# DK-Jang/MOCHA_SIGASIA2023

Hardware: AMD Instinct MI355X
Metric: characterized frames/sec (whole node) at T=60, 22 joints; 1/2/4/8 GPU (higher is better)
Workload: dtype f32; 1 GPU; demo pair (BASELINE configs[1]): 585 src x 585 cha windows, T=60, V=22, C=15, bank build + encode/match/decode/to_mot per step (characterize_pair); windows_per_gpu=585, joints=22, bank_entries=585, parallelism=dp1 (independent windows, no in-step collective)

## Files before the change

### mocha_sigasia2023_amd/csrc/gemm_x3.hip

```cpp
#include "kernels.h"
#include "device_utils.h"
#include <type_traits>
#include <algorithm>

namespace mocha {

typedef float f32x16 __attribute__((ext_vector_type(16)));
typedef float f32x4 __attribute__((ext_vector_type(4)));
typedef short s16x8 __attribute__((ext_vector_type(8)));
typedef unsigned int u32x2 __attribute__((ext_vector_type(2)));
typedef unsigned int u32x4 __attribute__((ext_vector_type(4)));

#ifndef X3_MAXSUM
#define X3_MAXSUM 2
#endif
static constexpr int XN = 128, XK = 16;
static constexpr int XA_HALF = 128 * 8 + 32;
static constexpr int XA_PLANE = 2 * XA_HALF;
static constexpr int XB_PLANE = 128 * 16;
static constexpr int XB_OFF = 3 * XA_PLANE;
static constexpr int X_STAGE = XB_OFF + 3 * XA_PLANE;
static constexpr int XW_BLOCK = 3 * XB_PLANE;
template <int TN> struct XT {
    static constexpr int TILE_N = 64 * TN;
    static constexpr int B_HALF = TILE_N * 8 + 32;
    static constexpr int B_PLANE = 2 * B_HALF;
    static constexpr int STAGE = XB_OFF + 3 * B_PLANE;
};
static_assert(XT<2>::STAGE == X_STAGE && XT<2>::B_HALF == XA_HALF, "TN = 2 is the 128-wide layout");

__device__ __forceinline__ float x3_lrelu(float x) { return x > 0.f ? x : 0.2f * x; }
__device__ __forceinline__ float x3_gelu(float x) { return mocha_gelu(x); }

__global__ __launch_bounds__(256) void mocha_pack_x3(const float* __restrict__ W, const float* __restrict__ wsub, int N, int K, unsigned short* __restrict__ out) {
    const int ksteps = K / XK;
    const int nt = blockIdx.x / ksteps, ks = blockIdx.x - nt * ksteps;
    const int r = threadIdx.x >> 1, h = threadIdx.x & 1;
    const int n = nt * XN + r;
    const int k = ks * XK + 8 * h;
    f32x4 lo = {0.f, 0.f, 0.f, 0.f}, hi = lo;
    if (n < N) {
        lo = *reinterpret_cast<const f32x4*>(W + (size_t)n * K + k);
        hi = *reinterpret_cast<const f32x4*>(W + (size_t)n * K + k + 4);
        if (wsub) {
            lo -= *reinterpret_cast<const f32x4*>(wsub + k);
            hi -= *reinterpret_cast<const f32x4*>(wsub + k + 4);
        }
    }
    u32x2 a[3], b[3];
    plane_split4(lo, a); plane_split4(hi, b);
    unsigned short* blk = out + (size_t)blockIdx.x * XW_BLOCK;
#pragma unroll
    for (int q = 0; q < 3; ++q) {
        const u32x4 v = {a[q][0], a[q][1], b[q][0], b[q][1]};
        *reinterpret_cast<u32x4*>(blk + q * XB_PLANE + h * 1024 + r * 8) = v;
    }
}

size_t gemm_x3_packed_elems(int N, int K) { return (size_t)((N + XN - 1) / XN) * (K / XK) * XW_BLOCK; }

hipError_t launch_pack_x3(const float* W, int N, int K, unsigned short* out, hipStream_t s, const float* wsub) {
    if (K % XK != 0) return hipErrorInvalidValue;
    const long long blocks = (long long)((N + XN - 1) / XN) * (K / XK);
    if (blocks > 0x7fffffffll) return hipErrorInvalidValue;
    hipLaunchKernelGGL(mocha_pack_x3, dim3((unsigned)blocks), dim3(256), 0, s, W, wsub, N, K, out);
    return hipGetLastError();
}

template <bool LRELU, bool GATHER, int TM, int TN>
__global__ __launch_bounds__(256) __attribute__((amdgpu_waves_per_eu(3, 3))) void mocha_gemm_x3(GemmParams p) {
    constexpr int TILE_M = TM * 64;
    constexpr int TILE_N = XT<TN>::TILE_N, B_HALF = XT<TN>::B_HALF, B_PLANE = XT<TN>::B_PLANE, STAGE = XT<TN>::STAGE;
    extern __shared__ __attribute__((aligned(16))) unsigned short x3_sm[];
    const int tid = threadIdx.x;
    const int lane = tid & 63, wave = tid >> 6;
    const int l31 = lane & 31, hh = lane >> 5;
    const int wm = wave >> 1, wn = wave & 1;

    const int n_tiles = (p.N + TILE_N - 1) / TILE_N;
    const int m_tiles = (p.M + TILE_M - 1) / TILE_M;
    const int bid = blockIdx.x;
    int mt, nt;
    if (m_tiles >= 8) {
        const int grp = bid / (8 * n_tiles);
        const int rem = bid - grp * 8 * n_tiles;
        mt = grp * 8 + (rem & 7);
        nt = rem >> 3;
    } else {
        mt = bid / n_tiles;
        nt = bid - mt * n_tiles;
    }
    if (mt >= m_tiles) return;
    const int m0 = mt * TILE_M, n0 = nt * TILE_N;
    const int steps_total = p.K / XK;
    const int per = (steps_total + p.ksplit - 1) / p.ksplit;
    const int s0 = blockIdx.z * per;
    const int nsteps = (s0 + per) <= steps_total ? per : steps_total - s0;
#ifdef X3_EXP_STAMPS
    long long stamp[4];
    stamp[3] = (long long)__builtin_amdgcn_s_memrealtime();
    stamp[0] = (long long)__builtin_amdgcn_s_memtime();
#define X3_STAMP(i) stamp[i] = (long long)__builtin_amdgcn_s_memtime()
#define X3_STAMP_OUT() do { if (tid == 0) { long long* d = (long long*)p.wsub + (size_t)bid * 6; d[0] = stamp[0]; d[1] = stamp[1]; d[2] = stamp[2]; d[3] = (long long)__builtin_amdgcn_s_memtime(); d[4] = stamp[3]; d[5] = (long long)__builtin_amdgcn_s_memrealtime(); } } while (0)
#else
#define X3_STAMP(i)
#define X3_STAMP_OUT()
#endif

    const int lrow = tid >> 2;
    const int lc = tid & 3;
    const __amdgpu_buffer_rsrc_t rsA = make_rsrc(GATHER ? p.A : p.A + (size_t)(m0 < p.M ? m0 : 0) * p.lda);
    int a_rb[TM], a_t[TM];
    unsigned a_off[TM];
#pragma unroll
    for (int i = 0; i < TM; ++i) {
        int m = m0 + lrow + 64 * i;
        m = m < p.M ? m : p.M - 1;
        if (GATHER) {
            const int v = m % p.V;
            const int bt = m / p.V;
            a_t[i] = bt % p.T_out;
            a_rb[i] = (bt / p.T_out) * p.T_src * p.V + v;
            a_off[i] = 0;
        } else {
            a_rb[i] = m; a_t[i] = 0;
            a_off[i] = ((unsigned)(m - m0) * (unsigned)p.lda + lc * 4) * 4u;
        }
    }
    f32x4 rset[2][TM];
    auto load_a = [&](int s, f32x4 (&ra)[TM]) __attribute__((always_inline)) {
        const int k0 = (s0 + s) * XK;
        if (!GATHER) {
#pragma unroll
            for (int i = 0; i < TM; ++i) ra[i] = bload(rsA, a_off[i], (unsigned)k0 * 4u);
        } else {
            const int tap = k0 / p.Cc;
            const int cin = k0 - tap * p.Cc;
#pragma unroll
            for (int i = 0; i < TM; ++i) {
                int tf = a_t[i] * p.stride + tap * p.tstep - p.pad;
                tf = tf < 0 ? -tf : tf;
                tf = tf >= p.T_full ? 2 * (p.T_full - 1) - tf : tf;
                const unsigned off = ((unsigned)(a_rb[i] + (tf >> p.tshift) * p.V) * (unsigned)p.lda + lc * 4) * 4u;
                ra[i] = bload(rsA, off, (unsigned)cin * 4u);
            }
        }
    };
    const int a_wr = (lc >> 1) * XA_HALF + lrow * 8 + (lc & 1) * 4;
    auto split_store = [&](const f32x4 (&ra)[TM], unsigned short* st) __attribute__((always_inline)) {
#pragma unroll
        for (int i = 0; i < TM; ++i) {
            f32x4 v = ra[i];
            if (LRELU) { v[0] = x3_lrelu(v[0]); v[1] = x3_lrelu(v[1]); v[2] = x3_lrelu(v[2]); v[3] = x3_lrelu(v[3]); }
            u32x2 pl[3];
            plane_split4(v, pl);
#pragma unroll
            for (int q = 0; q < 3; ++q) *reinterpret_cast<u32x2*>(st + q * XA_PLANE + a_wr + i * 64 * 8) = pl[q];
        }
    };
    const int wblock = TN == 1 ? nt >> 1 : nt;
    const __amdgpu_buffer_rsrc_t rsW = make_rsrc(p.Wsplit + ((size_t)wblock * steps_total + s0) * XW_BLOCK);
    auto dma_w = [&](int s, unsigned short* st) __attribute__((always_inline)) {
        if (TN == 2) {
#pragma unroll
            for (int j = 0; j < 3; ++j)
                __builtin_amdgcn_raw_ptr_buffer_load_lds(rsW, (__attribute__((address_space(3))) void*)(st + XB_OFF + ((j * 4 + wave) >> 2) * B_PLANE +
                                                         (((j * 4 + wave) >> 1) & 1) * B_HALF + ((j * 4 + wave) & 1) * 512), 16,
                                                         (unsigned)(j * 256 + tid) * 16u, (unsigned)s * (XW_BLOCK * 2u), 0, 0);
        } else {
#pragma unroll
            for (int j = 0; j < 2; ++j) {
                const int pc = j * 4 + wave;
                if (pc < 6)
                    __builtin_amdgcn_raw_ptr_buffer_load_lds(rsW, (__attribute__((address_space(3))) void*)(st + XB_OFF + (pc >> 1) * B_PLANE + (pc & 1) * B_HALF), 16,
                                                             (unsigned)(((pc >> 1) * 4 + (pc & 1) * 2 + (nt & 1)) * 64 + lane) * 16u, (unsigned)s * (XW_BLOCK * 2u), 0, 0);
            }
        }
    };

    f32x16 acc[TM][TN];
#pragma unroll
    for (int i = 0; i < TM; ++i)
#pragma unroll
        for (int j = 0; j < TN; ++j)
#pragma unroll
            for (int r = 0; r < 16; ++r) acc[i][j][r] = 0.f;

    const int fa = hh * XA_HALF + (wm * TM * 32 + l31) * 8;
    const int fb = XB_OFF + hh * B_HALF + (wn * 32 * TN + l31) * 8;

    load_a(0, rset[0]);
    __builtin_amdgcn_sched_barrier(0);
    dma_w(0, x3_sm);
    __builtin_amdgcn_sched_barrier(0);
    split_store(rset[0], x3_sm);
    load_a(1, rset[1]);
    __builtin_amdgcn_sched_barrier(0);
    asm volatile("s_waitcnt vmcnt(%0) lgkmcnt(0)\n\ts_barrier" ::"n"(TM) : "memory");

    auto step = [&](int s, auto parity, auto fetch_w, auto fetch_a) __attribute__((always_inline)) {
        constexpr bool FETCH_W = decltype(fetch_w)::value, FETCH_A = decltype(fetch_a)::value;
        constexpr int P = decltype(parity)::value;
        unsigned short* cur = x3_sm + P * STAGE;
        unsigned short* nxt = x3_sm + (P ^ 1) * STAGE;
        if (FETCH_W) dma_w(s + 1, nxt);
        __builtin_amdgcn_sched_barrier(0);
        if (FETCH_A) load_a(s + 2, rset[P]);
        __builtin_amdgcn_sched_barrier(0);
        s16x8 a[3][TM], b[3][TN];
        auto rd_a = [&](int q) __attribute__((always_inline)) {
#pragma unroll
            for (int i = 0; i < TM; ++i) a[q][i] = *reinterpret_cast<const s16x8*>(cur + q * XA_PLANE + fa + i * 32 * 8);
        };
        auto rd_b = [&](int q) __attribute__((always_inline)) {
#pragma unroll
            for (int i = 0; i < TN; ++i) b[q][i] = *reinterpret_cast<const s16x8*>(cur + q * B_PLANE + fb + i * 32 * 8);
        };
        rd_a(0); rd_b(2); rd_a(1); rd_b(1); rd_a(2); rd_b(0);
        float x[4 * TM];
        unsigned pk[2 * TM][3], hi[2 * TM][2];
        if (FETCH_W) {
#pragma unroll
            for (int e = 0; e < 4 * TM; ++e) { x[e] = rset[P ^ 1][e >> 2][e & 3]; if (LRELU) x[e] = fmaxf(x[e], 0.2f * x[e]); }
        }
        auto split_op = [&](int k) __attribute__((always_inline)) {
            const int pr = k / 11, o = k % 11, lvl = o / 5;
            float& x0 = x[2 * pr]; float& x1 = x[2 * pr + 1];
            if (o == 10) { pk[pr][2] = cvt_pk_bf16(x0, x1); return; }
            switch (o % 5) {
                case 0: pk[pr][lvl] = cvt_pk_bf16(x0, x1); break;
                case 1: hi[pr][0] = pk[pr][lvl] << 16; break;
                case 2: hi[pr][1] = pk[pr][lvl] & 0xffff0000u; break;
                case 3: x0 -= __uint_as_float(hi[pr][0]); break;
                default: x1 -= __uint_as_float(hi[pr][1]); break;
            }
        };
        auto write_row = [&](int i) __attribute__((always_inline)) {
#pragma unroll
            for (int q = 0; q < 3; ++q) {
                const u32x2 v = {pk[2 * i][q], pk[2 * i + 1][q]};
                *reinterpret_cast<u32x2*>(nxt + q * XA_PLANE + a_wr + i * 64 * 8) = v;
            }
        };
        __builtin_amdgcn_sched_barrier(0);
#pragma unroll
        for (int m = 0; m < 6 * TM * TN; ++m) {
            const int pr = m / (TM * TN), pa = PLANE_PA[pr], pb = PLANE_PB[pr], i = (m % (TM * TN)) / TN, j = m % TN;
            if (X3_MAXSUM == 2 || pr == 5)
                acc[i][j] = __builtin_amdgcn_mfma_f32_32x32x16_bf16(b[pb][j], a[pa][i], acc[i][j], 0, 0, 0);
            if (TN == 2) {
                if (FETCH_W && m < 11 * TM) { split_op(2 * m); split_op(2 * m + 1); }
                if (FETCH_W && m == 10) write_row(0);
                if (FETCH_W && TM == 2 && m == 21) write_row(1);
            } else if (TM == 1) {
                if (FETCH_W) {
#pragma unroll
                    for (int k = 4 * m; k < 4 * m + 4; ++k)
                        if (k < 22) split_op(k);
                }
                if (FETCH_W && m == 5) write_row(0);
            } else {
                if (FETCH_W && m < 11) { split_op(4 * m); split_op(4 * m + 1); split_op(4 * m + 2); split_op(4 * m + 3); }
                if (FETCH_W && m == 5) write_row(0);
                if (FETCH_W && m == 10) write_row(1);
            }
            __builtin_amdgcn_sched_barrier(0);
        }
        if (FETCH_A) asm volatile("s_waitcnt vmcnt(%0) lgkmcnt(0)\n\ts_barrier" ::"n"(TM) : "memory");
        else asm volatile("s_waitcnt vmcnt(0) lgkmcnt(0)\n\ts_barrier" ::: "memory");
    };
    X3_STAMP(1);
    using T = std::true_type; using F = std::false_type;
    using P0 = std::integral_constant<int, 0>; using P1 = std::integral_constant<int, 1>;
    for (int s = 0; s + 2 < nsteps; s += 2) {
        step(s, P0{}, T{}, T{});
        step(s + 1, P1{}, T{}, T{});
    }
    step(nsteps - 2, P0{}, T{}, F{});
    step(nsteps - 1, P1{}, F{}, F{});
    X3_STAMP(2);

    const bool vec_ok = ((p.ldc & 3) == 0) && (!p.residual || (p.ldr & 3) == 0) && ((p.N & 3) == 0);
    float* Cz = p.C + (size_t)blockIdx.z * p.slab_stride;
    const __amdgpu_buffer_rsrc_t rsC = make_rsrc(Cz + (size_t)m0 * p.ldc + n0);
    const __amdgpu_buffer_rsrc_t rsBias = make_rsrc(p.bias ? p.bias + n0 : p.A);
    const __amdgpu_buffer_rsrc_t rsRb = make_rsrc(p.rowbias ? p.rowbias + n0 : p.A);
    const __amdgpu_buffer_rsrc_t rsRes = make_rsrc(p.residual ? p.residual + (size_t)m0 * p.ldr + n0 : p.A);

    if (vec_ok && n0 + TILE_N <= p.N) {
        constexpr int LDP = TILE_N + 4;
        constexpr int C4 = TILE_N / 4;
        static_assert(64 * LDP * 4 <= 2 * STAGE * 2, "epilogue staging fits the operand stages");
        float* stage = reinterpret_cast<float*>(x3_sm);
        static_assert(256 % C4 == 0, "a thread keeps its column quad over the iterations");
        constexpr int NIT = 64 * C4 / 256, RSTEP = 256 / C4;
        const int c4 = tid % C4, r0 = tid / C4;
        const unsigned cb = (unsigned)c4 * 16u;
        const f32x4 zero4 = {0.f, 0.f, 0.f, 0.f};
        const f32x4 bias4 = p.bias ? bload(rsBias, cb, 0u) : zero4;
        const bool pre_res = p.residual != nullptr, pre_rb = !pre_res && p.rowbias != nullptr;
        f32x4 pre[2];
        auto fetch_pre = [&](int k) __attribute__((always_inline)) {
            const int rloc = 64 * (k / NIT) + r0 + RSTEP * (k % NIT);
            int row = m0 + rloc;
            row = row < p.M ? row : p.M - 1;
            if (pre_res) pre[k & 1] = bload(rsRes, (unsigned)(row - m0) * (unsigned)p.ldr * 4u + cb, 0u);
            else if (pre_rb) pre[k & 1] = bload(rsRb, (unsigned)(row % p.rb_mod) * (unsigned)p.N * 4u + cb, 0u);
        };
        if (pre_res || pre_rb) { fetch_pre(0); fetch_pre(1); }
        const bool plain_out = !p.bias && !p.rowbias && !p.residual;
#pragma unroll
        for (int h = 0; h < TM; ++h) {
#pragma unroll
            for (int i = 0; i < TM; ++i) {
                const int rblk = wm * TM + i;
                if ((rblk >> 1) != h) continue;
                float* srow = stage + ((rblk & 1) * 32 + l31) * LDP + wn * (32 * TN) + 4 * hh;
#pragma unroll
                for (int j = 0; j < TN; ++j)
#pragma unroll
                    for (int g = 0; g < 4; ++g) {
                        f32x4 v = {acc[i][j][4 * g], acc[i][j][4 * g + 1], acc[i][j][4 * g + 2], acc[i][j][4 * g + 3]};
                        *reinterpret_cast<f32x4*>(srow + j * 32 + 8 * g) = v;
                    }
            }
            __syncthreads();
            if (plain_out) {
#pragma unroll
                for (int it = 0; it < NIT; ++it) {
                    const int r = r0 + RSTEP * it;
                    const int rloc = 64 * h + r;
                    if (m0 + rloc < p.M) {
                        f32x4 v = *reinterpret_cast<const f32x4*>(stage + r * LDP + c4 * 4);
                        if (p.act == 1) { v = mocha_gelu4(v); }
                        else if (p.act == 2) { v[0] = x3_lrelu(v[0]); v[1] = x3_lrelu(v[1]); v[2] = x3_lrelu(v[2]); v[3] = x3_lrelu(v[3]); }
                        else if (p.act == 3) { v[0] = fmaxf(v[0], 0.f); v[1] = fmaxf(v[1], 0.f); v[2] = fmaxf(v[2], 0.f); v[3] = fmaxf(v[3], 0.f); }
                        bstore(rsC, v, (unsigned)rloc * (unsigned)p.ldc * 4u + cb, 0u);
                    }
                }
            } else
#pragma unroll
            for (int it = 0; it < NIT; ++it) {
                const int r = r0 + RSTEP * it;
                const int rloc = 64 * h + r;
                f32x4 v = *reinterpret_cast<const f32x4*>(stage + r * LDP + c4 * 4) + bias4;
                if (pre_rb) v += pre[(NIT * h + it) & 1];
                else if (p.rowbias) v += bload(rsRb, (unsigned)((m0 + rloc) % p.rb_mod) * (unsigned)p.N * 4u + cb, 0u);
                if (p.act == 1) { v = mocha_gelu4(v); }
                else if (p.act == 2) { v[0] = x3_lrelu(v[0]); v[1] = x3_lrelu(v[1]); v[2] = x3_lrelu(v[2]); v[3] = x3_lrelu(v[3]); }
                else if (p.act == 3) { v[0] = fmaxf(v[0], 0.f); v[1] = fmaxf(v[1], 0.f); v[2] = fmaxf(v[2], 0.f); v[3] = fmaxf(v[3], 0.f); }
                if (pre_res) v += pre[(NIT * h + it) & 1];
                if ((pre_res || pre_rb) && NIT * h + it + 2 < NIT * TM) fetch_pre(NIT * h + it + 2);
                if (m0 + rloc < p.M) bstore(rsC, v, (unsigned)rloc * (unsigned)p.ldc * 4u + cb, 0u);
            }
            if (h + 1 < TM) __syncthreads();
        }
        X3_STAMP_OUT();
        return;
    }

#pragma unroll
    for (int i = 0; i < TM; ++i) {
        const int row = m0 + (wm * TM + i) * 32 + l31;
        if (row >= p.M) continue;
        const float* rbrow = p.rowbias ? p.rowbias + (size_t)(row % p.rb_mod) * p.N : nullptr;
        const float* rsrow = p.residual ? p.residual + (size_t)row * p.ldr : nullptr;
        float* crow = Cz + (size_t)row * p.ldc;
#pragma unroll
        for (int j = 0; j < TN; ++j)
#pragma unroll
            for (int g = 0; g < 4; ++g)
#pragma unroll
                for (int e = 0; e < 4; ++e) {
                    const int c1 = n0 + wn * (32 * TN) + j * 32 + 8 * g + 4 * hh + e;
                    if (c1 >= p.N) continue;
                    float x = acc[i][j][4 * g + e];
                    if (p.bias) x += p.bias[c1];
                    if (rbrow) x += rbrow[c1];
                    if (p.act == 1) x = x3_gelu(x);
                    else if (p.act == 2) x = x3_lrelu(x);
                    else if (p.act == 3) x = fmaxf(x, 0.f);
                    if (rsrow) x += rsrow[c1];
                    crow[c1] = x;
                }
    }
}


template <bool LRELU, bool GATHER, int EPI>
__global__ __launch_bounds__(256) __attribute__((amdgpu_waves_per_eu(3, 3))) void mocha_gemm_x3p(GemmParams p) {
    constexpr int TM = 2, TN = 2;
    constexpr int TILE_M = 128, TILE_N = 128, B_HALF = XT<2>::B_HALF, B_PLANE = XT<2>::B_PLANE, STAGE = XT<2>::STAGE;
    extern __shared__ __attribute__((aligned(16))) unsigned short x3_sm[];
    const int tid = threadIdx.x;
    const int lane = tid & 63, wave = tid >> 6;
    const int l31 = lane & 31, hh = lane >> 5;
    const int wm = wave >> 1, wn = wave & 1;
    const int n_tiles = (p.N + TILE_N - 1) / TILE_N;
    const int m_tiles = (p.M + TILE_M - 1) / TILE_M;
    const int m_pad = m_tiles >= 8 ? (m_tiles + 7) / 8 * 8 : m_tiles;
    const int total = m_pad * n_tiles;
    const int nsteps = p.K / XK;
    const int lrow = tid >> 2, lc = tid & 3;

    struct Tile { int m0, n0; int valid; int a_rb[TM], a_t[TM]; unsigned a_off[TM]; };
    auto make_tile = [&](int t) __attribute__((always_inline)) -> Tile {
        Tile T;
        int mt, nt;
        if (m_tiles >= 8) {
            const int grp = t / (8 * n_tiles);
            const int rem = t - grp * 8 * n_tiles;
            mt = grp * 8 + (rem & 7);
            nt = rem >> 3;
        } else {
            mt = t / n_tiles;
            nt = t - mt * n_tiles;
        }
        T.valid = mt < m_tiles;
        T.m0 = (T.valid ? mt : 0) * TILE_M; T.n0 = nt * TILE_N;
#pragma unroll
        for (int i = 0; i < TM; ++i) {
            int m = T.m0 + lrow + 64 * i;
            m = m < p.M ? m : p.M - 1;
            if (GATHER) {
                const int v = m % p.V;
                const int bt = m / p.V;
                T.a_t[i] = bt % p.T_out;
                T.a_rb[i] = (bt / p.T_out) * p.T_src * p.V + v;
                T.a_off[i] = 0;
            } else {
                T.a_rb[i] = m; T.a_t[i] = 0;
                T.a_off[i] = ((unsigned)(m - T.m0) * (unsigned)p.lda + lc * 4) * 4u;
            }
        }
        return T;
    };
    f32x4 rset[2][TM];
    auto load_a = [&](const Tile& T, int s, f32x4 (&ra)[TM]) __attribute__((always_inline)) {
        const __amdgpu_buffer_rsrc_t rsA = make_rsrc(GATHER ? p.A : p.A + (size_t)T.m0 * p.lda);
        const int k0 = s * XK;
        if (!GATHER) {
#pragma unroll
            for (int i = 0; i < TM; ++i) ra[i] = bload(rsA, T.a_off[i], (unsigned)k0 * 4u);
        } else {
            const int tap = k0 / p.Cc;
            const int cin = k0 - tap * p.Cc;
#pragma unroll
            for (int i = 0; i < TM; ++i) {
                int tf = T.a_t[i] * p.stride + tap * p.tstep - p.pad;
                tf = tf < 0 ? -tf : tf;
                tf = tf >= p.T_full ? 2 * (p.T_full - 1) - tf : tf;
                const unsigned off = ((unsigned)(T.a_rb[i] + (tf >> p.tshift) * p.V) * (unsigned)p.lda + lc * 4) * 4u;
                ra[i] = bload(rsA, off, (unsigned)cin * 4u);
            }
        }
    };
    const int a_wr = (lc >> 1) * XA_HALF + lrow * 8 + (lc & 1) * 4;
    auto split_store = [&](const f32x4 (&ra)[TM], unsigned short* st) __attribute__((always_inline)) {
#pragma unroll
        for (int i = 0; i < TM; ++i) {
            f32x4 v = ra[i];
            if (LRELU) { v[0] = x3_lrelu(v[0]); v[1] = x3_lrelu(v[1]); v[2] = x3_lrelu(v[2]); v[3] = x3_lrelu(v[3]); }
            u32x2 pl[3];
            plane_split4(v, pl);
#pragma unroll
            for (int q = 0; q < 3; ++q) *reinterpret_cast<u32x2*>(st + q * XA_PLANE + a_wr + i * 64 * 8) = pl[q];
        }
    };
    auto dma_w = [&](const Tile& T, int s, unsigned short* st) __attribute__((always_inline)) {
        const __amdgpu_buffer_rsrc_t rsW = make_rsrc(p.Wsplit + ((size_t)(T.n0 / TILE_N) * nsteps) * XW_BLOCK);
#pragma unroll
        for (int j = 0; j < 3; ++j)
            __builtin_amdgcn_raw_ptr_buffer_load_lds(rsW, (__attribute__((address_space(3))) void*)(st + XB_OFF + ((j * 4 + wave) >> 2) * B_PLANE +
                                                     (((j * 4 + wave) >> 1) & 1) * B_HALF + ((j * 4 + wave) & 1) * 512), 16,
                                                     (unsigned)(j * 256 + tid) * 16u, (unsigned)s * (XW_BLOCK * 2u), 0, 0);
    };

    f32x16 acc[TM][TN];
    const int fa = hh * XA_HALF + (wm * TM * 32 + l31) * 8;
    const int fb = XB_OFF + hh * B_HALF + (wn * 32 * TN + l31) * 8;

    auto step = [&](auto parity, auto fetch_w, auto fetch_a, const Tile& wt, int ws, const Tile& at, int as) __attribute__((always_inline)) {
        constexpr bool FETCH_W = decltype(fetch_w)::value, FETCH_A = decltype(fetch_a)::value;
        constexpr int P = decltype(parity)::value;
        unsigned short* cur = x3_sm + P * STAGE;
        unsigned short* nxt = x3_sm + (P ^ 1) * STAGE;
        if (FETCH_W) dma_w(wt, ws, nxt);
        __builtin_amdgcn_sched_barrier(0);
        if (FETCH_A) load_a(at, as, rset[P]);
        __builtin_amdgcn_sched_barrier(0);
        s16x8 a[3][TM], b[3][TN];
        auto rd_a = [&](int q) __attribute__((always_inline)) {
#pragma unroll
            for (int i = 0; i < TM; ++i) a[q][i] = *reinterpret_cast<const s16x8*>(cur + q * XA_PLANE + fa + i * 32 * 8);
        };
        auto rd_b = [&](int q) __attribute__((always_inline)) {
#pragma unroll
            for (int i = 0; i < TN; ++i) b[q][i] = *reinterpret_cast<const s16x8*>(cur + q * B_PLANE + fb + i * 32 * 8);
        };
        rd_a(0); rd_b(2); rd_a(1); rd_b(1); rd_a(2); rd_b(0);
        float x[4 * TM];
        unsigned pk[2 * TM][3], hi[2 * TM][2];
        if (FETCH_W) {
#pragma unroll
            for (int e = 0; e < 4 * TM; ++e) { x[e] = rset[P ^ 1][e >> 2][e & 3]; if (LRELU) x[e] = fmaxf(x[e], 0.2f * x[e]); }
        }
        auto split_op = [&](int k) __attribute__((always_inline)) {
            const int pr = k / 11, o = k % 11, lvl = o / 5;
            float& x0 = x[2 * pr]; float& x1 = x[2 * pr + 1];
            if (o == 10) { pk[pr][2] = cvt_pk_bf16(x0, x1); return; }
            switch (o % 5) {
                case 0: pk[pr][lvl] = cvt_pk_bf16(x0, x1); break;
                case 1: hi[pr][0] = pk[pr][lvl] << 16; break;
                case 2: hi[pr][1] = pk[pr][lvl] & 0xffff0000u; break;
                case 3: x0 -= __uint_as_float(hi[pr][0]); break;
                default: x1 -= __uint_as_float(hi[pr][1]); break;
            }
        };
        auto write_row = [&](int i) __attribute__((always_inline)) {
#pragma unroll
            for (int q = 0; q < 3; ++q) {
                const u32x2 v = {pk[2 * i][q], pk[2 * i + 1][q]};
                *reinterpret_cast<u32x2*>(nxt + q * XA_PLANE + a_wr + i * 64 * 8) = v;
            }
        };
        __builtin_amdgcn_sched_barrier(0);
#pragma unroll
        for (int m = 0; m < 6 * TM * TN; ++m) {
            const int pr = m / (TM * TN), pa = PLANE_PA[pr], pb = PLANE_PB[pr], i = (m % (TM * TN)) / TN, j = m % TN;
            acc[i][j] = __builtin_amdgcn_mfma_f32_32x32x16_bf16(b[pb][j], a[pa][i], acc[i][j], 0, 0, 0);
            if (FETCH_W && m < 11 * TM) { split_op(2 * m); split_op(2 * m + 1); }
            if (FETCH_W && m == 10) write_row(0);
            if (FETCH_W && m == 21) write_row(1);
            __builtin_amdgcn_sched_barrier(0);
        }
        if (FETCH_A) asm volatile("s_waitcnt vmcnt(%0) lgkmcnt(0)\n\ts_barrier" ::"n"(TM) : "memory");
        else asm volatile("s_waitcnt vmcnt(0) lgkmcnt(0)\n\ts_barrier" ::: "memory");
    };
    using TT = std::true_type;
    using P0 = std::integral_constant<int, 0>; using P1 = std::integral_constant<int, 1>;

    int t = blockIdx.x;
    if (t >= total) return;
    Tile cur = make_tile(t);
    while (!cur.valid) { t += gridDim.x; if (t >= total) return; cur = make_tile(t); }
    load_a(cur, 0, rset[0]);
    __builtin_amdgcn_sched_barrier(0);
    dma_w(cur, 0, x3_sm);
    __builtin_amdgcn_sched_barrier(0);
    split_store(rset[0], x3_sm);
    load_a(cur, 1, rset[1]);
    __builtin_amdgcn_sched_barrier(0);
    asm volatile("s_waitcnt vmcnt(%0) lgkmcnt(0)\n\ts_barrier" ::"n"(TM) : "memory");

    const bool vec_ok = ((p.ldc & 3) == 0) && (!p.residual || (p.ldr & 3) == 0) && ((p.N & 3) == 0);
    for (;;) {
        int tn = t + gridDim.x;
        Tile nxt = cur;
        bool has_next = false;
        while (tn < total) { nxt = make_tile(tn); if (nxt.valid) { has_next = true; break; } tn += gridDim.x; }
#pragma unroll
        for (int i = 0; i < TM; ++i)
#pragma unroll
            for (int j = 0; j < TN; ++j)
#pragma unroll
                for (int r = 0; r < 16; ++r) acc[i][j][r] = 0.f;
        for (int s = 0; s + 2 < nsteps; s += 2) {
            step(P0{}, TT{}, TT{}, cur, s + 1, cur, s + 2);
            step(P1{}, TT{}, TT{}, cur, s + 2, cur, s + 3);
        }
        step(P0{}, TT{}, TT{}, cur, nsteps - 1, nxt, 0);
        step(P1{}, TT{}, TT{}, nxt, 0, nxt, 1);

        const int m0 = cur.m0, n0 = cur.n0;
        float* Cz = p.C;
        const __amdgpu_buffer_rsrc_t rsC = make_rsrc(Cz + (size_t)m0 * p.ldc + n0);
        const __amdgpu_buffer_rsrc_t rsBias = make_rsrc(p.bias ? p.bias + n0 : p.A);
        const __amdgpu_buffer_rsrc_t rsRb = make_rsrc(p.rowbias ? p.rowbias + n0 : p.A);
        const __amdgpu_buffer_rsrc_t rsRes = make_rsrc(p.residual ? p.residual + (size_t)m0 * p.ldr + n0 : p.A);
        if (vec_ok && n0 + TILE_N <= p.N) {
            constexpr int LDP = TILE_N + 4;
            constexpr int C4 = TILE_N / 4;
            static_assert(32 * LDP * 4 <= STAGE * 2, "a 32-row pass fits one stage");
            float* stage = reinterpret_cast<float*>(x3_sm + STAGE);
            int te = tid, l31e = l31, hhe = hh;
            asm volatile("" : "+v"(te), "+v"(l31e), "+v"(hhe));
            static_assert(256 % C4 == 0, "a thread keeps its column quad over the iterations");
            constexpr int NIT = 32 * C4 / 256;
            const int c4 = te % C4, r0 = te / C4;
            const unsigned cb = (unsigned)c4 * 16u;
            const f32x4 zero4 = {0.f, 0.f, 0.f, 0.f};
            const f32x4 bias4 = p.bias ? bload(rsBias, cb, 0u) : zero4;
            f32x4 pre[EPI ? 2 : 1];
            auto fetch_pre = [&](int k) __attribute__((always_inline)) {
                const int rloc = 32 * (k / NIT) + r0 + (256 / C4) * (k % NIT);
                int row = m0 + rloc;
                row = row < p.M ? row : p.M - 1;
                if constexpr (EPI == 1) pre[k & 1] = bload(rsRes, (unsigned)(row - m0) * (unsigned)p.ldr * 4u + cb, 0u);
                else if constexpr (EPI == 2) pre[k & 1] = bload(rsRb, (unsigned)(row % p.rb_mod) * (unsigned)p.N * 4u + cb, 0u);
            };
            if constexpr (EPI != 0) { fetch_pre(0); fetch_pre(1); }
#pragma unroll
            for (int h = 0; h < 2 * TM; ++h) {
#pragma unroll
                for (int i = 0; i < TM; ++i) {
                    if (wm * TM + i != h) continue;
                    float* srow = stage + l31e * LDP + wn * (32 * TN) + 4 * hhe;
#pragma unroll
                    for (int j = 0; j < TN; ++j)
#pragma unroll
                        for (int g = 0; g < 4; ++g) {
                            f32x4 v = {acc[i][j][4 * g], acc[i][j][4 * g + 1], acc[i][j][4 * g + 2], acc[i][j][4 * g + 3]};
                            *reinterpret_cast<f32x4*>(srow + j * 32 + 8 * g) = v;
                        }
                }
                __syncthreads();
                if (EPI == 0 && !p.bias) {
#pragma unroll
                    for (int it = 0; it < NIT; ++it) {
                        const int rloc = 32 * h + r0 + (256 / C4) * it;
                        if (m0 + rloc < p.M) {
                            f32x4 v = *reinterpret_cast<const f32x4*>(stage + (r0 + (256 / C4) * it) * LDP + c4 * 4);
                            if (p.act == 1) { v = mocha_gelu4(v); }
                            else if (p.act == 2) { v[0] = x3_lrelu(v[0]); v[1] = x3_lrelu(v[1]); v[2] = x3_lrelu(v[2]); v[3] = x3_lrelu(v[3]); }
                            else if (p.act == 3) { v[0] = fmaxf(v[0], 0.f); v[1] = fmaxf(v[1], 0.f); v[2] = fmaxf(v[2], 0.f); v[3] = fmaxf(v[3], 0.f); }
                            bstore(rsC, v, (unsigned)rloc * (unsigned)p.ldc * 4u + cb, 0u);
                        }
                    }
                } else
#pragma unroll
                for (int it = 0; it < NIT; ++it) {
                    const int rloc = 32 * h + r0 + (256 / C4) * it;
                    f32x4 v = *reinterpret_cast<const f32x4*>(stage + (r0 + (256 / C4) * it) * LDP + c4 * 4) + bias4;
                    if constexpr (EPI == 2) v += pre[(NIT * h + it) & 1];
                    else if (EPI == 1 && p.rowbias) v += bload(rsRb, (unsigned)((m0 + rloc) % p.rb_mod) * (unsigned)p.N * 4u + cb, 0u);
                    if (p.act == 1) { v = mocha_gelu4(v); }
                    else if (p.act == 2) { v[0] = x3_lrelu(v[0]); v[1] = x3_lrelu(v[1]); v[2] = x3_lrelu(v[2]); v[3] = x3_lrelu(v[3]); }
                    else if (p.act == 3) { v[0] = fmaxf(v[0], 0.f); v[1] = fmaxf(v[1], 0.f); v[2] = fmaxf(v[2], 0.f); v[3] = fmaxf(v[3], 0.f); }
                    if constexpr (EPI == 1) v += pre[(NIT * h + it) & 1];
                    if constexpr (EPI != 0) { if (NIT * h + it + 2 < NIT * 2 * TM) fetch_pre(NIT * h + it + 2); }
                    if (m0 + rloc < p.M) bstore(rsC, v, (unsigned)rloc * (unsigned)p.ldc * 4u + cb, 0u);
                }
                __syncthreads();
            }
        } else {
#pragma unroll
            for (int i = 0; i < TM; ++i) {
                const int row = m0 + (wm * TM + i) * 32 + l31;
                if (row >= p.M) continue;
                const float* rbrow = p.rowbias ? p.rowbias + (size_t)(row % p.rb_mod) * p.N : nullptr;
                const float* rsrow = p.residual ? p.residual + (size_t)row * p.ldr : nullptr;
                float* crow = Cz + (size_t)row * p.ldc;
#pragma unroll
                for (int j = 0; j < TN; ++j)
#pragma unroll
                    for (int g = 0; g < 4; ++g)
#pragma unroll
                        for (int e = 0; e < 4; ++e) {
                            const int c1 = n0 + wn * (32 * TN) + j * 32 + 8 * g + 4 * hh + e;
                            if (c1 >= p.N) continue;
                            float x = acc[i][j][4 * g + e];
                            if (p.bias) x += p.bias[c1];
                            if (rbrow) x += rbrow[c1];
                            if (p.act == 1) x = x3_gelu(x);
                            else if (p.act == 2) x = x3_lrelu(x);
                            else if (p.act == 3) x = fmaxf(x, 0.f);
                            if (rsrow) x += rsrow[c1];
                            crow[c1] = x;
                        }
            }
        }
        if (!has_next) break;
        cur = nxt; t = tn;
    }
}

template <int TN> static constexpr size_t x3_lds_bytes() { return (size_t)2 * XT<TN>::STAGE * sizeof(unsigned short); }

template <bool L, bool G, int TM, int TN>
static hipError_t x3_attr() {
    return hipFuncSetAttribute(reinterpret_cast<const void*>(&mocha_gemm_x3<L, G, TM, TN>), hipFuncAttributeMaxDynamicSharedMemorySize, (int)x3_lds_bytes<TN>());
}

hipError_t gemm_x3_init() {
    hipError_t e = x3_attr<false, false, 2, 2>();
    if (e == hipSuccess) e = x3_attr<true, false, 2, 2>();
    if (e == hipSuccess) e = x3_attr<false, true, 2, 2>();
    if (e == hipSuccess) e = x3_attr<true, true, 2, 2>();
    if (e == hipSuccess) e = x3_attr<false, false, 1, 2>();
    if (e == hipSuccess) e = x3_attr<true, false, 1, 2>();
    if (e == hipSuccess) e = x3_attr<false, true, 1, 2>();
    if (e == hipSuccess) e = x3_attr<true, true, 1, 2>();
    if (e == hipSuccess) e = x3_attr<false, false, 2, 1>();
    if (e == hipSuccess) e = x3_attr<true, false, 2, 1>();
    if (e == hipSuccess) e = x3_attr<false, true, 2, 1>();
    if (e == hipSuccess) e = x3_attr<true, true, 2, 1>();
    if (e == hipSuccess) e = x3_attr<false, false, 1, 1>();
    if (e == hipSuccess) e = x3_attr<true, false, 1, 1>();
    if (e == hipSuccess) e = x3_attr<false, true, 1, 1>();
    if (e == hipSuccess) e = x3_attr<true, true, 1, 1>();
    if (e == hipSuccess) e = hipFuncSetAttribute(reinterpret_cast<const void*>(&mocha_gemm_x3p<false, false, 0>), hipFuncAttributeMaxDynamicSharedMemorySize, (int)x3_lds_bytes<2>());
    if (e == hipSuccess) e = hipFuncSetAttribute(reinterpret_cast<const void*>(&mocha_gemm_x3p<false, false, 1>), hipFuncAttributeMaxDynamicSharedMemorySize, (int)x3_lds_bytes<2>());
    if (e == hipSuccess) e = hipFuncSetAttribute(reinterpret_cast<const void*>(&mocha_gemm_x3p<false, false, 2>), hipFuncAttributeMaxDynamicSharedMemorySize, (int)x3_lds_bytes<2>());
    if (e == hipSuccess) e = hipFuncSetAttribute(reinterpret_cast<const void*>(&mocha_gemm_x3p<true, false, 0>), hipFuncAttributeMaxDynamicSharedMemorySize, (int)x3_lds_bytes<2>());
    if (e == hipSuccess) e = hipFuncSetAttribute(reinterpret_cast<const void*>(&mocha_gemm_x3p<true, false, 1>), hipFuncAttributeMaxDynamicSharedMemorySize, (int)x3_lds_bytes<2>());
    if (e == hipSuccess) e = hipFuncSetAttribute(reinterpret_cast<const void*>(&mocha_gemm_x3p<true, false, 2>), hipFuncAttributeMaxDynamicSharedMemorySize, (int)x3_lds_bytes<2>());
    if (e == hipSuccess) e = hipFuncSetAttribute(reinterpret_cast<const void*>(&mocha_gemm_x3p<false, true, 0>), hipFuncAttributeMaxDynamicSharedMemorySize, (int)x3_lds_bytes<2>());
    if (e == hipSuccess) e = hipFuncSetAttribute(reinterpret_cast<const void*>(&mocha_gemm_x3p<false, true, 1>), hipFuncAttributeMaxDynamicSharedMemorySize, (int)x3_lds_bytes<2>());
    if (e == hipSuccess) e = hipFuncSetAttribute(reinterpret_cast<const void*>(&mocha_gemm_x3p<false, true, 2>), hipFuncAttributeMaxDynamicSharedMemorySize, (int)x3_lds_bytes<2>());
    if (e == hipSuccess) e = hipFuncSetAttribute(reinterpret_cast<const void*>(&mocha_gemm_x3p<true, true, 0>), hipFuncAttributeMaxDynamicSharedMemorySize, (int)x3_lds_bytes<2>());
    if (e == hipSuccess) e = hipFuncSetAttribute(reinterpret_cast<const void*>(&mocha_gemm_x3p<true, true, 1>), hipFuncAttributeMaxDynamicSharedMemorySize, (int)x3_lds_bytes<2>());
    if (e == hipSuccess) e = hipFuncSetAttribute(reinterpret_cast<const void*>(&mocha_gemm_x3p<true, true, 2>), hipFuncAttributeMaxDynamicSharedMemorySize, (int)x3_lds_bytes<2>());
    return e;
}

static bool x3_tile64(const GemmParams& p) {
    if (p.ksplit > 1 || p.N % 64 != 0 || !gemm_is_small(p)) return false;
    if (p.N % XN != 0) return true;
    const long long t64x128 = (long long)((p.M + 63) / 64) * ((p.N + 127) / 128);
    return t64x128 < p.tile64_below;
}

bool gemm_x3_supports(const GemmParams& p) {
#ifndef X3_EXP_STAMPS
    if (p.wsub) return false;
#endif
    if (p.K % (2 * XK) != 0) return false;
    if (p.gather && (p.R != 1 || p.Cc % XK != 0)) return false;
    if (p.ksplit > 1) {
        if (p.bias || p.rowbias || p.residual || p.act || p.gather) return false;
        const int total = p.K / XK, per = (total + p.ksplit - 1) / p.ksplit;
        if ((per & 1) || total - (p.ksplit - 1) * per < 2 || ((total - (p.ksplit - 1) * per) & 1)) return false;
        return (long long)total * XW_BLOCK * 2 < (1ll << 31);
    }
    if (p.N % 64 != 0) return false;
    if (p.N % XN != 0 && gemm_is_small(p) && !x3_tile64(p)) return false;
    if (gemm_is_skinny(p)) return false;
    return true;
}

template <int TM, int TN>
static void x3_launch(const GemmParams& p, hipStream_t s) {
    const int m_tiles = (p.M + TM * 64 - 1) / (TM * 64);
    const int m_pad = m_tiles >= 8 ? (m_tiles + 7) / 8 * 8 : m_tiles;
    const dim3 grid(m_pad * ((p.N + 64 * TN - 1) / (64 * TN)), 1, p.ksplit > 1 ? p.ksplit : 1);
    if (p.a_lrelu) {
        if (p.gather) hipLaunchKernelGGL((mocha_gemm_x3<true, true, TM, TN>), grid, dim3(256), x3_lds_bytes<TN>(), s, p);
        else hipLaunchKernelGGL((mocha_gemm_x3<true, false, TM, TN>), grid, dim3(256), x3_lds_bytes<TN>(), s, p);
    } else {
        if (p.gather) hipLaunchKernelGGL((mocha_gemm_x3<false, true, TM, TN>), grid, dim3(256), x3_lds_bytes<TN>(), s, p);
        else hipLaunchKernelGGL((mocha_gemm_x3<false, false, TM, TN>), grid, dim3(256), x3_lds_bytes<TN>(), s, p);
    }
}


hipError_t launch_gemm_x3(const GemmParams& p, hipStream_t s) {
    if (p.M <= 0 || p.N <= 0) return hipSuccess;
    if (!p.Wsplit || !gemm_x3_supports(p)) return hipErrorInvalidValue;
    if (p.gather && (long long)p.M / p.T_out * p.T_src * p.lda * 4 >= (1ll << 31)) return hipErrorInvalidValue;
    if (128ll * p.lda * 4 >= (1ll << 31)) return hipErrorInvalidValue;
    if (p.persistent > 0 && p.ksplit <= 1 && p.N % XN == 0 && p.N <= p.persistent_max_n && !gemm_is_small(p)) {
        const int m_tiles = (p.M + 127) / 128, m_pad = m_tiles >= 8 ? (m_tiles + 7) / 8 * 8 : m_tiles;
        const long long total = (long long)m_pad * (p.N / XN);
        const unsigned grid = (unsigned)std::min<long long>(total, p.persistent);
        const int epi = p.residual ? 1 : p.rowbias ? 2 : 0;
#define X3P_LAUNCH(L, G)                                                                                                                  \
        do {                                                                                                                              \
            if (epi == 1) hipLaunchKernelGGL((mocha_gemm_x3p<L, G, 1>), dim3(grid), dim3(256), x3_lds_bytes<2>(), s, p);                 \
            else if (epi == 2) hipLaunchKernelGGL((mocha_gemm_x3p<L, G, 2>), dim3(grid), dim3(256), x3_lds_bytes<2>(), s, p);            \
            else hipLaunchKernelGGL((mocha_gemm_x3p<L, G, 0>), dim3(grid), dim3(256), x3_lds_bytes<2>(), s, p);                          \
        } while (0)
        if (p.a_lrelu) { if (p.gather) X3P_LAUNCH(true, true); else X3P_LAUNCH(true, false); }
        else { if (p.gather) X3P_LAUNCH(false, true); else X3P_LAUNCH(false, false); }
#undef X3P_LAUNCH
        return hipGetLastError();
    }
    if (x3_tile64(p)) x3_launch<1, 1>(p, s);
    else if (p.ksplit <= 1 && p.N % XN != 0) x3_launch<2, 1>(p, s);
    else if (p.ksplit <= 1 && gemm_is_small(p)) x3_launch<1, 2>(p, s);
    else x3_launch<2, 2>(p, s);
    return hipGetLastError();
}

}
```

### mocha_sigasia2023_amd/csrc/kernels.h

```cpp
#pragma once
#include <hip/hip_runtime.h>
#include <stdint.h>

namespace mocha {

struct GemmParams {
    const float* A = nullptr;
    const float* W = nullptr;
    const float* wsub = nullptr;
    const unsigned short* Wsplit = nullptr;
    float* C = nullptr;
    const float* bias = nullptr;
    const float* rowbias = nullptr;
    const float* residual = nullptr;
    int M = 0, N = 0, K = 0;
    int lda = 0, ldc = 0, ldr = 0;
    int rb_mod = 1;
    int act = 0;
    int a_lrelu = 0;
    int gather = 0;
    int T_out = 1, V = 1, ntaps = 1, pad = 0, stride = 1, R = 1, T_full = 1, tshift = 0, Cc = 0, T_src = 1;
    int tstep = 1;
    float ascale = 1.f;
    int ksplit = 1;
    long long slab_stride = 0;
    int persistent = 768, persistent_max_n = 512;
    int tile64_below = 0;
    const unsigned short* Wh2 = nullptr;
    const float* w_inv = nullptr;
    const float* a_amax = nullptr;
    float* c_amax = nullptr;
    int rows_per_win = 0;
};
hipError_t launch_gemm(const GemmParams& p, hipStream_t s);
bool gemm_is_narrow(const GemmParams& p);
bool gemm_is_small(const GemmParams& p);
bool gemm_is_skinny(const GemmParams& p);
bool gemm_is_skinny16(const GemmParams& p);
hipError_t gemm_init();
hipError_t gemm_x3_init();
bool gemm_x3_supports(const GemmParams& p);
size_t gemm_x3_packed_elems(int N, int K);
hipError_t launch_pack_x3(const float* W, int N, int K, unsigned short* out, hipStream_t s, const float* wsub = nullptr);
hipError_t launch_gemm_x3(const GemmParams& p, hipStream_t s);
hipError_t gemm_x3r_init();
bool gemm_x3r_supports(const GemmParams& p);
hipError_t launch_gemm_x3r(const GemmParams& p, hipStream_t s, int grid = 0);
hipError_t gemm_h2_init();
bool gemm_h2_supports(const GemmParams& p);
size_t gemm_h2_packed_elems(int N, int K);
hipError_t launch_pack_h2(const float* W, int N, int K, unsigned short* out, float* w_inv , hipStream_t s);
hipError_t launch_gemm_h2(const GemmParams& p, hipStream_t s);
hipError_t launch_absmax(const float* x, long long nwin, long long per, float* out , hipStream_t s, float mul = 1.f, float add = 0.f);
hipError_t launch_gather_f32(const float* table, const int32_t* idx, long long rows, float* out, int n, hipStream_t s);


struct AttnParams {
    const float* q; const float* k; const float* v; float* out;
    int ldq, ldk, ldv, ldo;
    int B, heads, dh, nq, nk;
    float scale;
    int hsk = -1, hsv = -1;
    int split_max = 192;
    const int32_t* kv_idx = nullptr; long long kv_rows = 0;
};
hipError_t launch_attention(const AttnParams& p, hipStream_t s);
hipError_t launch_attention_x3(const AttnParams& p, hipStream_t s);
hipError_t attention_x3_init();
static constexpr int ATTN_KV_STAGE_BYTES = 3 * 96 * 64;
static constexpr int ATTN_KV_IMG_BYTES = 16 * ATTN_KV_STAGE_BYTES;
struct AttnKvParams {
    const float* q; float* out; const unsigned short* kv;
    int ldq, ldo;
    int B, heads, dh, nq, nk;
    float scale;
    int pairs = 0;
};
hipError_t launch_attention_x3_kv(const AttnKvParams& p, hipStream_t s);

hipError_t launch_embed_front(const float* X, const float* W1, const float* b1, const float* AP ,
                              float* out, int nframes, int V, int Cin, const float* xmean, const float* xstd, int raw_root,
                              hipStream_t s, bool planes = false, int max_wgs = 512);
hipError_t launch_embed_sums(const float* X, const float* W1, const float* b1, const float* AP, float* u, int nwin, int V, int Cin,
                             const float* xmean, const float* xstd, int raw_root, hipStream_t s, int max_wgs = 512);
hipError_t launch_body_front(const float* x, const float* A_b , float* out, int rows6 , hipStream_t s);
hipError_t launch_joint_expand(const float* g, const float* AU , float* out, int nframes15, int V, hipStream_t s);
hipError_t launch_final_proj(const float* z, const float* W6, const float* b6, float* Y, int rows, int Cout, int V,
                             const float* ymean, const float* ystd, hipStream_t s, int phased = 0);
static constexpr int QSTAT_PARTS = 4;
struct InormExtra {
    const float* centre = nullptr; float* zc = nullptr;
    unsigned short* zc16 = nullptr;
    long long plane_stride = 0; float* qstat = nullptr;
    const float* table = nullptr; const int32_t* row_idx = nullptr; long long table_rows = 0; float* copy_out = nullptr;
    unsigned short* kvimg = nullptr;
    int split_max = 1 << 30;
    double* mean64 = nullptr;
};
hipError_t launch_instnorm(const float* x, float* out, float* mean_out, const float* gm, const float* gs, float* zn,
                           int B, int n, hipStream_t s, const InormExtra* ex = nullptr);
hipError_t launch_adain(const float* x, const float* gb, int gb_stride , float* xad, float* qin, int B, int n, hipStream_t s,
                        int closed = 1, const int32_t* gb_idx = nullptr, long long gb_rows = 0, int split_max = 1 << 30);
hipError_t launch_linear_f64(const double* X, int ldx, int xcol, const double* W, const double* bias, double* y64, float* y32, int ldy,
                             int M, int N, int K, int L, int act, hipStream_t s);
hipError_t launch_window_sums(const float* y, float* u, int rows, int channels , hipStream_t s);
hipError_t launch_layernorm256(const float* x, const float* w, const float* b, float* y, int rows, hipStream_t s);
hipError_t launch_cvae_prior_tokens(const float* c, const float* mu_tok, const float* lv_tok, const float* pe, float* out, int B, int nc, hipStream_t s);
hipError_t launch_cvae_latent(const float* x , int ntok, const float* eps, const float* c, int nc, const float* pe, int nq,
                              float* mem, float* q, float* mu_out, float* logvar_out, int B, hipStream_t s);
hipError_t launch_cvae_condition(const float* src_cnt, const float* sm, const float* ss, const float* prev, const float* cm,
                                 const float* cs, float* cond, int B, int n, hipStream_t s);
hipError_t launch_scale_shift(const float* x, const float* mean, const float* sd, float* out, int B, int n, hipStream_t s);
hipError_t featurize_init();
hipError_t launch_featurize(const float* Yrot, const float* Ypos, const float* Yvel, const float* Yang, const int* parents ,
                            float* X, int B, int T, int J, hipStream_t s);
static constexpr int LIVE_WINDOW = 60;
struct LiveRing { int32_t* counters; float *rot, *pos, *vel, *ang; };
hipError_t live_init();
hipError_t launch_live_push(const LiveRing& r, const float* Yrot, const float* Ypos, const float* Yvel, const float* Yang, const int32_t* seg,
                            const int* parents , float* X, int32_t* eff, int32_t* valid, int S, int J, hipStream_t s);
#define MOCHA_MAX_CONTACT 4
#define MOCHA_MAX_CHAIN 8
#define MOCHA_MAX_BONES 32
static constexpr int POST_STATE_DOUBLES = 8 + MOCHA_MAX_BONES * 3 + MOCHA_MAX_CONTACT * 19;
struct PostParams {
    const float* heads;
    const float* speed;
    const float* src_rvel;
    const float* src_rang;
    const float* src_speed;
    const unsigned char* contact;
    double *pos, *rot, *ik_rot;
    double *bvh_pos, *bvh_euler;
    int n_clips, n_frames, V, n_contact, ik_enabled, blend_enabled;
    int parents[MOCHA_MAX_BONES];
    int contact_bones[MOCHA_MAX_CONTACT];
    double dt, max_length_buffer, foot_height, unlock_radius, halflife;
    double* state;
    const int32_t* valid;
};
hipError_t launch_pose_heads(const float* Y, float* heads, float* speed, int B, int T, int V, hipStream_t s);
hipError_t launch_post_clip(const PostParams& p, hipStream_t s);
hipError_t launch_post_step(const PostParams& p, hipStream_t s);
size_t column_mean_scratch_doubles(int cols);
hipError_t launch_column_mean(const float* x, int64_t N, int cols, float* mean, double* scratch, hipStream_t s);
hipError_t launch_column_stats(const float* x, int64_t N, int cols, float* mean, float* sd, hipStream_t s);
hipError_t launch_rownorm2(const float* x, const float* sub , float* out, int64_t rows, int cols, hipStream_t s);
hipError_t launch_sub_rows(const float* x, const float* sub, float* out, int64_t rows, int cols, hipStream_t s);
hipError_t match_mfma_init();
int match_bf16_ksplit(int Q, int64_t N);
hipError_t launch_center_bf16(const float* x, const float* centre, void* out, int64_t rows, int cols, hipStream_t s);
hipError_t launch_center_rows(const float* x, const float* centre, void* planes, int nplanes, float* out32, float* qstat, int64_t rows, int cols, hipStream_t s);
hipError_t launch_match_gemm_bf16(const void* qc16, const void* bank16, float* S, int Q, int64_t N, int D, int ksplit, hipStream_t s, int planes = 1,
                                  const void* tiled = nullptr, int nt_bank = 0, unsigned* tickets = nullptr);
int match_pass256_ksplit(int Q, int64_t N);
hipError_t launch_match_pass256(const void* qc16, const void* bank16, float* S, int Q, int64_t N, int D, int ksplit, hipStream_t s, int variant = 0,
                                int planes = 1, const void* tiled32 = nullptr);
size_t match_tile32_elems(int64_t N, int D);
hipError_t launch_tile32_bf16(const void* bank16, void* out, int64_t N, int D, hipStream_t s);
size_t match_tiled_elems(int64_t N, int D);
hipError_t launch_tile_bf16(const void* bank16, void* out, int64_t N, int D, hipStream_t s);
hipError_t launch_match_select(const float* S, int ksplit, long long slab_stride, int lds, const float* bnorm, const float* query,
                               const float* centre, const float* bank, const void* bank16, float margin_rel, int Q, int64_t N, int D,
                               int32_t* idx, float* dist, hipStream_t s);
hipError_t launch_match_select2(const float* S, int ksplit, long long slab_stride, int lds, const float* bnorm, const float* query,
                                const float* centre, const float* bank, const void* bank16, const float* qstat, float margin_rel, int Q,
                                int64_t N, int D, int32_t* idx, float* dist, hipStream_t s);
size_t match_stream_scratch(int Q, int64_t N);
hipError_t launch_match_stream(const void* bank, int bank_bf16, const float* query, int Q, int64_t N, int D,
                               unsigned long long* partial, int32_t* idx, float* dist, hipStream_t s);
hipError_t launch_match_topk(const void* bank, int bank_bf16, const float* query, int Q, int64_t N, int D, int k,
                             unsigned long long* keys, int32_t* idx, float* dist, hipStream_t s);
hipError_t launch_gather_blend(const float* src, const int32_t* idx, const float* dist, float temperature, float* out, int Q, int k,
                               int cols, int64_t nrows, hipStream_t s);
hipError_t launch_to_bf16(const float* x, const float* sub , int cols, void* y, int64_t n, hipStream_t s);
hipError_t match_refine_init();
size_t match_scan16_scratch_words(int64_t N);
size_t match_scan16_scratch_head_words();
hipError_t launch_to_i8(const float* x, const float* centre, void* y, float* scale, float* rho, int64_t rows, int cols, hipStream_t s);
hipError_t match_scan8_init();
size_t match_scan8_mode_word();
hipError_t launch_match_scan8(const void* bank8, const float* scale8, const float* rho8, const void* bank16, const float* rho16, const float* bank,
                              const float* qc, const float* query, int Q, int64_t N, int D, unsigned long long* scratch, int32_t* idx, float* dist, hipStream_t s);
hipError_t launch_match_refine(const unsigned long long* keys, const unsigned long long* wgmin, int nwg, const float* rho16, const float* rho8, unsigned* mode,
                               const float* bank, const float* query, int nq, int64_t N, int D, int32_t* idx, float* dist, unsigned long long* scratch, hipStream_t s);
hipError_t launch_rowresid(const float* x, const float* centre, const void* x16, float* rho, int64_t rows, int cols, hipStream_t s);
hipError_t launch_match_scan16(const void* bank16, const float* rho, const float* bank, const float* qc, const float* query, int Q, int64_t N,
                               int D, unsigned long long* scratch, int32_t* idx, float* dist, hipStream_t s);
hipError_t launch_rownorm2_bf16(const void* x, float* out, int64_t rows, int cols, hipStream_t s);
static constexpr int SEG_MAX_Q = 4096;
size_t match_seg_scratch_words(int Q, int64_t max_rows);
size_t seg_plan_ints(int Q, int S);
hipError_t launch_match_segmented(const void* bank, int bank_bf16, const float* query, const int32_t* seg, int Q, const int* seg_start, int S,
                                  int64_t max_rows, int D, unsigned long long* partial, int* plan, int32_t* idx, int32_t* gidx, float* dist,
                                  hipStream_t s);
hipError_t launch_gather_rows(const float* src, const int32_t* idx, float* out, int Q, int cols, int64_t nrows, hipStream_t s);

}
```

Baseline: 113,400 frames/s.

## Split persistent GEMM tail tiles into 64x64 sub-tile launch for load balance

When the persistent 128x128 GEMM has a partial final wave of tiles (remainder up to tail_max), the persistent kernel now processes only the full waves. A second launch handles the leftover 128-tiles, with each one split into four 64x64 sub-tiles on the non-persistent kernel. This targets wave-quantization imbalance, where a few CUs would otherwise process a lone extra tile. It adds a second kernel launch and uses the smaller-tile path for the tail, which reuses data less.

```diff
diff --git a/mocha_sigasia2023_amd/csrc/gemm_x3.hip b/mocha_sigasia2023_amd/csrc/gemm_x3.hip
--- a/mocha_sigasia2023_amd/csrc/gemm_x3.hip
+++ b/mocha_sigasia2023_amd/csrc/gemm_x3.hip
@@ -81,7 +81,24 @@
     const int m_tiles = (p.M + TILE_M - 1) / TILE_M;
     const int bid = blockIdx.x;
     int mt, nt;
-    if (m_tiles >= 8) {
+    if (TM == 1 && TN == 1 && p.tile_count > 0) {
+        const int tl = (bid >> 5) * 8 + (bid & 7), sub = (bid >> 3) & 3;
+        if (tl >= p.tile_count) return;
+        const int t = p.tile_first + tl;
+        const int n128 = p.N / XN, m128 = (p.M + 127) / 128;
+        int mt2, nt2;
+        if (m128 >= 8) {
+            const int grp = t / (8 * n128);
+            const int rem = t - grp * 8 * n128;
+            mt2 = grp * 8 + (rem & 7);
+            nt2 = rem >> 3;
+        } else {
+            mt2 = t / n128;
+            nt2 = t - mt2 * n128;
+        }
+        mt = 2 * mt2 + (sub >> 1);
+        nt = 2 * nt2 + (sub & 1);
+    } else if (m_tiles >= 8) {
         const int grp = bid / (8 * n_tiles);
         const int rem = bid - grp * 8 * n_tiles;
         mt = grp * 8 + (rem & 7);
@@ -399,7 +416,7 @@
     const int n_tiles = (p.N + TILE_N - 1) / TILE_N;
     const int m_tiles = (p.M + TILE_M - 1) / TILE_M;
     const int m_pad = m_tiles >= 8 ? (m_tiles + 7) / 8 * 8 : m_tiles;
-    const int total = m_pad * n_tiles;
+    const int total = p.tile_count > 0 ? p.tile_count : m_pad * n_tiles;
     const int nsteps = p.K / XK;
     const int lrow = tid >> 2, lc = tid & 3;
 
@@ -764,15 +781,30 @@
         const long long total = (long long)m_pad * (p.N / XN);
         const unsigned grid = (unsigned)std::min<long long>(total, p.persistent);
         const int epi = p.residual ? 1 : p.rowbias ? 2 : 0;
+        const long long rem = total % grid;
+        const bool tail = total > grid && rem > 0 && rem <= p.tail_max;
+        GemmParams pw = p;
+        pw.tile_first = 0; pw.tile_count = tail ? (int)(total - rem) : 0;
 #define X3P_LAUNCH(L, G)                                                                                                                  \
         do {                                                                                                                              \
-            if (epi == 1) hipLaunchKernelGGL((mocha_gemm_x3p<L, G, 1>), dim3(grid), dim3(256), x3_lds_bytes<2>(), s, p);                 \
-            else if (epi == 2) hipLaunchKernelGGL((mocha_gemm_x3p<L, G, 2>), dim3(grid), dim3(256), x3_lds_bytes<2>(), s, p);            \
-            else hipLaunchKernelGGL((mocha_gemm_x3p<L, G, 0>), dim3(grid), dim3(256), x3_lds_bytes<2>(), s, p);                          \
+            if (epi == 1) hipLaunchKernelGGL((mocha_gemm_x3p<L, G, 1>), dim3(grid), dim3(256), x3_lds_bytes<2>(), s, pw);                \
+            else if (epi == 2) hipLaunchKernelGGL((mocha_gemm_x3p<L, G, 2>), dim3(grid), dim3(256), x3_lds_bytes<2>(), s, pw);           \
+            else hipLaunchKernelGGL((mocha_gemm_x3p<L, G, 0>), dim3(grid), dim3(256), x3_lds_bytes<2>(), s, pw);                         \
         } while (0)
         if (p.a_lrelu) { if (p.gather) X3P_LAUNCH(true, true); else X3P_LAUNCH(true, false); }
         else { if (p.gather) X3P_LAUNCH(false, true); else X3P_LAUNCH(false, false); }
 #undef X3P_LAUNCH
+        if (tail) {
+            pw.tile_first = (int)(total - rem); pw.tile_count = (int)rem;
+            const dim3 tgrid((unsigned)((rem + 7) / 8 * 32));
+            if (p.a_lrelu) {
+                if (p.gather) hipLaunchKernelGGL((mocha_gemm_x3<true, true, 1, 1>), tgrid, dim3(256), x3_lds_bytes<1>(), s, pw);
+                else hipLaunchKernelGGL((mocha_gemm_x3<true, false, 1, 1>), tgrid, dim3(256), x3_lds_bytes<1>(), s, pw);
+            } else {
+                if (p.gather) hipLaunchKernelGGL((mocha_gemm_x3<false, true, 1, 1>), tgrid, dim3(256), x3_lds_bytes<1>(), s, pw);
+                else hipLaunchKernelGGL((mocha_gemm_x3<false, false, 1, 1>), tgrid, dim3(256), x3_lds_bytes<1>(), s, pw);
+            }
+        }
         return hipGetLastError();
     }
     if (x3_tile64(p)) x3_launch<1, 1>(p, s);
diff --git a/mocha_sigasia2023_amd/csrc/kernels.h b/mocha_sigasia2023_amd/csrc/kernels.h
--- a/mocha_sigasia2023_amd/csrc/kernels.h
+++ b/mocha_sigasia2023_amd/csrc/kernels.h
@@ -25,6 +25,8 @@
     int ksplit = 1;
     long long slab_stride = 0;
     int persistent = 768, persistent_max_n = 512;
+    int tail_max = 192;
+    int tile_first = 0, tile_count = 0;
     int tile64_below = 0;
     const unsigned short* Wh2 = nullptr;
     const float* w_inv = nullptr;
```

Result: slower. 109,200 frames/s (-3.7%).
